# martinambrus/PitchExtractor

Measured on AMD Instinct MI355X. Metric: mel-frames/sec training throughput (JDCNet, 24 kHz, batch=256), higher is better.
Workload: dtype f32

## Files before the change

### pitchextractor_amd/csrc/conv.hip

```cpp
#include <type_traits>
#include "splitk.h"

namespace {
using namespace pe;
typedef unsigned int u32x4_t __attribute__((ext_vector_type(4)));
typedef unsigned int u32x2_t __attribute__((ext_vector_type(2)));

__global__ void repack3x3_kernel(const float* __restrict__ w, float* __restrict__ w_fwd,
                                 float* __restrict__ w_dgrad, int Cout, int Cin) {
  const int idx = blockIdx.x * blockDim.x + threadIdx.x;
  if (idx >= Cout * Cin * 9) return;
  const int tap = idx % 9, ci = (idx / 9) % Cin, co = idx / (9 * Cin);
  const float v = w[idx];
  if (w_fwd) w_fwd[((long)co * 9 + tap) * Cin + ci] = v;
  if (w_dgrad) w_dgrad[((long)ci * 9 + (8 - tap)) * Cout + co] = v;
}

__global__ void transpose2d_kernel(const float* __restrict__ in, float* __restrict__ out, int rows, int cols) {
  __shared__ float tile[32][33];
  const int c0 = blockIdx.x * 32, r0 = blockIdx.y * 32;
  for (int i = threadIdx.y; i < 32; i += 8) {
    const int r = r0 + i, c = c0 + threadIdx.x;
    tile[i][threadIdx.x] = (r < rows && c < cols) ? in[(long)r * cols + c] : 0.f;
  }
// ... 62 lines not shown
template <int NT, class TH = __bf16>
__global__ void wfrag_pack_kernel(const float* __restrict__ w, long ld, int N, int K, uint4* __restrict__ out,
                                  const unsigned* __restrict__ amax = nullptr) {
  const long idx = (long)blockIdx.x * blockDim.x + threadIdx.x;
  const int NB32 = (N + 31) >> 5, KB = K >> 4;
  const int lane = (int)(idx & 63);
  const long blk = idx >> 6;
  if (blk >= (long)NB32 * KB) return;
  const int nb = (int)(blk % NB32), kb = (int)(blk / NB32);
  const int n = nb * 32 + (lane & 31), k = kb * 16 + (lane >> 5) * 8;
  float4 v0 = make_float4(0.f, 0.f, 0.f, 0.f), v1 = v0;
  if (n < N) {
    v0 = *reinterpret_cast<const float4*>(w + (long)n * ld + k);
    v1 = *reinterpret_cast<const float4*>(w + (long)n * ld + k + 4);
  }
  uint4* dst = out + ((long)(kb * NB32 + nb) * NT) * 64 + lane;
  if constexpr (NT == 3) {
    const Split3 a = split3(v0), b = split3(v1);
    dst[0] = make_uint4(a.hi.x, a.hi.y, b.hi.x, b.hi.y);
    dst[64] = make_uint4(a.mid.x, a.mid.y, b.mid.x, b.mid.y);
    dst[128] = make_uint4(a.lo.x, a.lo.y, b.lo.x, b.lo.y);
  } else if constexpr (NT == 2) {
    const float sc = h2_scale(*amax);
    const Split2 a = split2(v0, sc), b = split2(v1, sc);
    dst[0] = make_uint4(a.hi.x, a.hi.y, b.hi.x, b.hi.y);
    dst[64] = make_uint4(a.lo.x, a.lo.y, b.lo.x, b.lo.y);
  } else {
    const half4<TH> a = to_half4<TH>(v0), b = to_half4<TH>(v1);
    const uint2 ua = __builtin_bit_cast(uint2, a), ub = __builtin_bit_cast(uint2, b);
    dst[0] = make_uint4(ua.x, ua.y, ub.x, ub.y);
  }
}

template <int BN, int MODE, int PASSES, int D, bool FA2, class TA = float, class TH = __bf16>
__global__ __launch_bounds__(256, 2) void conv3x3_halo_wf_kernel(const TA* __restrict__ x,
                                                                 const uint4* __restrict__ wf, ConvEpiT<TA> ep, int T,
                                                                 int F, int C, int N, int P, int tiles_m,
                                                                 int tiles_n, const unsigned* amax_x,
                                                                 const unsigned* amax_w) {
  constexpr int NT = mode_terms<MODE>();
  using H = term_t<NT, TH>;
  H2Scales hs{1.f, 1.f, 1.f};
  if constexpr (MODE == kSplit2) hs.load(amax_x, amax_w);
  constexpr int TM = 2, TN = BN / 64, WN = BN / 2;
  constexpr int ZR = PASSES * 32;
  constexpr int AIMG = (ZR + 4) * 32;
  constexpr int S = 18 * TN;
  static_assert(S % D == 0 && D >= 2, "the fragment ring wraps at chunk boundaries");
  __shared__ __attribute__((aligned(16))) H As[NT * AIMG];
  const int tid = threadIdx.x, lane = tid & 63, wv = tid >> 6;
  const int wm = wv >> 1, wn = wv & 1, r = lane & 31, h = lane >> 5;
  const int tile = xcd_remap(blockIdx.x, tiles_m * tiles_n);
  const int p0 = (tile / tiles_n) * 128, n0 = (tile % tiles_n) * BN;
  const int WR = 128 + 2 * F + 2;
  const int srow = tid >> 3, piece = tid & 7;
  const int nchunks = C / 32;

  unsigned vbits[TM];
#pragma unroll
  for (int i = 0; i < TM; ++i) {
    const int p = p0 + wm * 64 + i * 32 + r;
    unsigned b = 0;
    if (p < P) {
      const int f = p % F, t = (p / F) % T;
#pragma unroll
      for (int tap = 0; tap < 9; ++tap) {
        const int tt = t + tap / 3 - 1, ff = f + tap % 3 - 1;
        if (tt >= 0 && tt < T && ff >= 0 && ff < F) b |= 1u << tap;
      }
    }
    vbits[i] = b;
  }

  typedef typename RawQuad<TA>::type Raw;
  Raw ra[PASSES];
  const __amdgpu_buffer_rsrc_t xrs = __builtin_amdgcn_make_buffer_rsrc(
      const_cast<TA*>(x), 0, (unsigned)((long)P * C * (long)sizeof(TA)), 0x00020000);
  unsigned voa[PASSES];
#pragma unroll
  for (int ps = 0; ps < PASSES; ++ps) {
    const int wr = ps * 32 + srow;
    const long q = (long)p0 - F - 1 + wr;
    voa[ps] = (wr < WR && q >= 0 && q < P) ? (unsigned)((q * C + piece * 4) * (long)sizeof(TA)) : 0x80000000u;
  }
  auto fetch_a = [&](int cc) {
    const unsigned so = (unsigned)(cc * 32 * (int)sizeof(TA));
#pragma unroll
// ... 138 lines not shown
#pragma unroll
        for (int g = 0; g < 16; ++g) {
          const int row = row0 + i * 32 + (g & 3) + 8 * (g >> 2), col = n0 + wn * WN + j * 32 + r;
          if (row < ep.rows && col < ep.N) {
            TA* d = ep.Y + (long)row * ep.N + col;
            float v = MODE == kSplit2 ? hs.unscale(acc[i][j][g]) : acc[i][j][g];
            if (ep.accumulate) v += ld1(d);
            st1(d, v);
            if (stats) add_stat(j, row, v);
          }
        }
  };
  if (!ep.buffer) epilogue_pointer();
  else if (ep.accumulate) epilogue_buffer(std::true_type{});
  else epilogue_buffer(std::false_type{});
  if (ep.stats) {
#pragma unroll
    for (int j = 0; j < TN; ++j) {
      s1[j] += __shfl_xor(s1[j], 32, 64);
      s2[j] += __shfl_xor(s2[j], 32, 64);
    }
    __syncthreads();
    double* red = reinterpret_cast<double*>(As);
    if (h == 0) {
#pragma unroll
      for (int j = 0; j < TN; ++j) {
        red[(wm * BN + wn * WN + j * 32 + r) * 2] = s1[j];
        red[(wm * BN + wn * WN + j * 32 + r) * 2 + 1] = s2[j];
      }
    }
    __syncthreads();
    const long tile_m = tile / tiles_n;
    for (int c = tid; c < BN; c += 256) {
      if (n0 + c < ep.N) {
        ep.stats[(tile_m * 2) * ep.N + n0 + c] = red[c * 2] + red[(BN + c) * 2];
        ep.stats[(tile_m * 2 + 1) * ep.N + n0 + c] = red[c * 2 + 1] + red[(BN + c) * 2 + 1];
      }
    }
  }
}

template <int BN, class FM, int PASSES, int D, bool FA2, class TA = typename FM::TA>
int launch_conv_halo_wf(const TA* x, const void* wf, TA* y, int B, int T, int F, int C, int N, int accumulate,
                        double* stats, hipStream_t st, const unsigned* amax_x, const unsigned* amax_w) {
  const int P = B * T * F;
  ConvEpiT<TA> ep{y, P, N, accumulate, stats, pe_epilogue_buffer((long)(P + 128) * N * (long)sizeof(TA))};
  const int tm = pe_cdiv(P, 128), tn = pe_cdiv(N, BN);
  hipLaunchKernelGGL((conv3x3_halo_wf_kernel<BN, FM::MODE, PASSES, D, FA2, TA, typename FM::TH>), dim3(tm * tn),
                     dim3(256), 0, st, x, reinterpret_cast<const uint4*>(wf), ep, T, F, C, N, P, tm, tn, amax_x, amax_w);
  PE_LAUNCH_CHECK();
  return PE_OK;
}

static inline size_t pe_wfrag_bytes_host(int N, int K, int terms) { return (size_t)((N + 31) / 32) * (K / 16) * terms * 1024; }

int conv_halo_passes(int F, int N) {
  const int wr = 128 + 2 * F + 2;
  if (wr <= 7 * 32 && N >= 96) return 7;
  if (wr <= 10 * 32 && N <= 64) return 10;
  return 0;
}

template <int BM, int BN>
__global__ __launch_bounds__(256) void conv3x3_wgrad_kernel(const float* __restrict__ dy, const float* __restrict__ x,
                                                            float* __restrict__ ws, int T, int F, int Cin,
                                                            int Cout, int P, int k_per_split, int tiles_n,
                                                            int n_tiles, int n_chunks) {
  __shared__ __attribute__((aligned(16))) float As[kBK * BM];
  __shared__ __attribute__((aligned(16))) float Bs[kBK * BN];
  const int xcd = blockIdx.x & 7, q = blockIdx.x >> 3;
  const int tap = q % 9;
  const int chunk = (q / 9) * 8 + xcd;
  if (chunk >= n_chunks) return;
  const int tile = chunk % n_tiles, split = chunk / n_tiles;
  const int m0 = (tile / tiles_n) * BM, n0 = (tile % tiles_n) * BN;
  const int kb = split * k_per_split;
  const int ke = min(P, kb + k_per_split);
  KRowLoader<BM> al{dy, (long)Cout, Cout, 0};
  ShiftedPixelLoader<BN> bl;
  bl.p = x; bl.T = T; bl.F = F; bl.C = Cin; bl.dt = tap / 3 - 1; bl.df = tap % 3 - 1;
  al.init(m0, kb);
  bl.init(n0, kb);
  f32x16 acc[BM / 64][BN / 64];
  tn_zero_acc<BM, BN>(acc);
  tn_mainloop<BM, BN>(al, bl, kb, ke, As, Bs, acc);
  float* dst = ws + ((long)split * 9 + tap) * Cout * Cin;
  tn_for_each_acc<BM, BN>(acc, [&](int r, int c, float v) {
    const int co = m0 + r, ci = n0 + c;
    if (co < Cout && ci < Cin) dst[(long)co * Cin + ci] = v;
  });
}

template <int DUMMY>
// ... 525 lines not shown
  if ((K & 15) || (ld & 3)) return PE_E_UNSUPPORTED;
  const long threads = (long)((N + 31) / 32) * (K / 16) * 64;
  hipLaunchKernelGGL((wfrag_pack_kernel<TERMS, typename FM::TH>), dim3(pe_cdiv(threads, 256)), dim3(256), 0,
                     pe_stream(stream), w, ld, N, K, reinterpret_cast<uint4*>(out), TERMS == 2 ? amax : nullptr);
  PE_LAUNCH_CHECK();
  return PE_OK;
}

extern "C" int pe_wfrag_pack(int products, const float* w, long ld, int N, int K, const unsigned* amax, void* wfrag,
                             void* stream) {
  return with_form<kTermForms, false>(products, 0, [&](auto f) {
    return wfrag_pack_impl<decltype(f)>(w, ld, N, K, amax, wfrag, stream);
  });
}

extern "C" int pe_conv3x3_wf_supported(int F, int C, int N) {
  return (C % 32) == 0 && conv_halo_passes(F, N) != 0 ? 1 : 0;
}

extern "C" int pe_conv3x3_wf_stat_parts(int B, int T, int F) { return pe_cdiv((long)B * T * F, 128); }

template <class FM, class TA = typename FM::TA>
static int conv3x3_fwd_wf_impl(const TA* x, const void* wfrag, TA* y, int B, int T, int F, int C, int N,
                               int accumulate, double* stats, void* stream, const unsigned* amax_x,
                               const unsigned* amax_w) {
  constexpr int MODE = FM::MODE;
  if (!x || !wfrag || !y || B <= 0 || T <= 0 || F <= 0 || C <= 0 || N <= 0) return PE_E_ARG;
  if ((C % 32) != 0 || (long)B * T * F * (C > N ? C : N) >= (1L << 31)) return PE_E_UNSUPPORTED;
  if ((long)B * T * F * C * (long)sizeof(TA) >= (1L << 31) || (long)pe_wfrag_bytes_host(N, 9 * C, mode_terms<MODE>()) >= (1L << 31))
    return PE_E_UNSUPPORTED;
  if (MODE == kSplit2 && (!amax_x || !amax_w)) return PE_E_ARG;
  hipStream_t st = pe_stream(stream);
  const int passes = conv_halo_passes(F, N);
  if (passes == 10)
    return launch_conv_halo_wf<64, FM, 10, 6, true>(x, wfrag, y, B, T, F, C, N, accumulate, stats, st, amax_x, amax_w);
  if (passes == 7) {
    if (N % 192 == 0 && N % 128 != 0)
      return launch_conv_halo_wf<192, FM, 7, 3, false>(x, wfrag, y, B, T, F, C, N, accumulate, stats, st, amax_x,
                                                       amax_w);
    return launch_conv_halo_wf<128, FM, 7, 3, true>(x, wfrag, y, B, T, F, C, N, accumulate, stats, st, amax_x, amax_w);
  }
  return PE_E_UNSUPPORTED;
}

extern "C" int pe_conv3x3_fwd_wf(int products, int act16, const void* x, const void* wfrag, void* y, int B, int T, int F,
                                 int C, int N, int accumulate, double* bn_partials, const unsigned* amax_x,
                                 const unsigned* amax_w, void* stream) {
  return with_form<kTermForms, true>(products, act16, [&](auto f) {
    using TA = typename decltype(f)::TA;
    return conv3x3_fwd_wf_impl<decltype(f)>(static_cast<const TA*>(x), wfrag, static_cast<TA*>(y), B, T, F, C, N,
                                            accumulate, bn_partials, stream, amax_x, amax_w);
  });
}

extern "C" size_t pe_conv3x3_wgrad_workspace_bytes(int B, int T, int F, int Cin, int Cout) {
  if (Cin == 1) return (size_t)kC1WgradBlocks * 576 * sizeof(float);
  return (size_t)wgrad_plan(B * T * F, Cout, Cin).k.splits * 9 * Cout * Cin * sizeof(float);
}

template <class FM, class TA = typename FM::TA>
static int conv3x3_wgrad_impl(const TA* x, const TA* dy, float* dw_oihw, int B, int T, int F, int Cin,
                              int Cout, float* workspace, size_t workspace_bytes, void* stream,
                              const unsigned* amax_x, const unsigned* amax_dy) {
  constexpr int MODE = FM::MODE;
  using TH = typename FM::TH;
  if (!x || !dy || !dw_oihw || B <= 0 || T <= 0 || F <= 0 || Cin <= 0 || Cout <= 0) return PE_E_ARG;
  if (MODE == kSplit2 && (!amax_x || !amax_dy)) return PE_E_ARG;
  if ((Cin & 3) || (Cout & 3)) return PE_E_UNSUPPORTED;
// ... 114 lines not shown
```

### pitchextractor_amd/csrc/elementwise.hip

```cpp
#include <type_traits>
#include "forms.h"

namespace {
using namespace pe;

constexpr int kMaxPartials = 4096;

template <class F>
__device__ __forceinline__ void column_reduce2(F&& f, long n_pix, int C, double* partial ) {
  extern __shared__ __attribute__((aligned(16))) char smem_raw[];
  double* red = reinterpret_cast<double*>(smem_raw);
  const int quads = C >> 2;
  const int G = 256 / quads;
  const int q = threadIdx.x % quads, g = threadIdx.x / quads;
  double s1[4] = {0, 0, 0, 0}, s2[4] = {0, 0, 0, 0};
  if (g < G) {
    for (long p = (long)blockIdx.x * G + g; p < n_pix; p += (long)gridDim.x * G) {
      float4 a, b;
      f(p, q * 4, a, b);
      s1[0] += a.x; s1[1] += a.y; s1[2] += a.z; s1[3] += a.w;
      s2[0] += b.x; s2[1] += b.y; s2[2] += b.z; s2[3] += b.w;
    }
#pragma unroll
    for (int i = 0; i < 4; ++i) {
      red[(g * 2 + 0) * C + q * 4 + i] = s1[i];
      red[(g * 2 + 1) * C + q * 4 + i] = s2[i];
    }
  }
  __syncthreads();
  for (int i = threadIdx.x; i < 2 * C; i += 256) {
    double s = 0;
    for (int gg = 0; gg < G; ++gg) s += red[gg * 2 * C + i];
    partial[(long)blockIdx.x * 2 * C + i] = s;
  }
}

__device__ __forceinline__ float lrelu(float v, float slope) { return v > 0.f ? v : v * slope; }

template <class TA>
__global__ __launch_bounds__(256) void bn_stats_partial_kernel(const TA* __restrict__ x, long n_pix, int C,
                                                               double* __restrict__ partial) {
  column_reduce2(
      [&](long p, int c, float4& a, float4& b) {
        a = ld4(x + p * C + c);
        b = make_float4(a.x * a.x, a.y * a.y, a.z * a.z, a.w * a.w);
      },
      n_pix, C, partial);
}

__global__ __launch_bounds__(256) void bn_partials_fold_kernel(const double* __restrict__ partial, int nparts, int C2,
                                                               double* __restrict__ out) {
  for (int col = threadIdx.x; col < C2; col += 256) {
    double s = 0.0;
    for (int p = blockIdx.x; p < nparts; p += gridDim.x) s += partial[(long)p * C2 + col];
    out[(long)blockIdx.x * C2 + col] = s;
  }
}

__global__ void bn_stats_finalize_kernel(const double* __restrict__ partial, int nparts, long n_pix, int C,
                                         const float* __restrict__ gamma, const float* __restrict__ beta, float eps,
                                         float momentum, float* __restrict__ running_mean,
                                         float* __restrict__ running_var, float* __restrict__ mean_out,
                                         float* __restrict__ invstd_out, float* __restrict__ scale,
                                         float* __restrict__ shift) {
  const int c = blockIdx.x * 4 + (threadIdx.x >> 6);
  if (c >= C) return;
  const double s1 = pe_wave_strided_sum(partial + c, 2L * C, nparts);
// ... 248 lines not shown
__global__ __launch_bounds__(256) void bn_bwd_apply_kernel(const BnBwdArgs a, const float* __restrict__ c1,
                                                           const float* __restrict__ c2, float* __restrict__ dx,
                                                           unsigned* __restrict__ amax) {
  const int quads = a.C >> 2;
  const long total = a.n_in_pix * quads;
  float am = 0.f;
  for (long i = (long)blockIdx.x * 256 + threadIdx.x; i < total; i += (long)gridDim.x * 256) {
    const int c = (int)(i % quads) * 4;
    const long p = i / quads;
    const float4 dz = dz_quad(a, p, c);
    const float4 v = *reinterpret_cast<const float4*>(a.x + p * a.C + c);
    const float4 mu = *reinterpret_cast<const float4*>(a.mean + c);
    const float4 is = *reinterpret_cast<const float4*>(a.invstd + c);
    const float4 sc = *reinterpret_cast<const float4*>(a.scale + c);
    const float4 k1 = bn_term(c1, c), k2 = bn_term(c2, c);
    float4 o;
    o.x = sc.x * (dz.x - k1.x - (v.x - mu.x) * is.x * k2.x);
    o.y = sc.y * (dz.y - k1.y - (v.y - mu.y) * is.y * k2.y);
    o.z = sc.z * (dz.z - k1.z - (v.z - mu.z) * is.z * k2.z);
    o.w = sc.w * (dz.w - k1.w - (v.w - mu.w) * is.w * k2.w);
    *reinterpret_cast<float4*>(dx + p * a.C + c) = o;
    am = amax4(am, o);
  }
  amax_commit(am, amax);
}

template <int POOL>
struct BnWindow {
  float4 v[POOL], dz[POOL];
  long p0;
  int n;
};

template <int POOL, class TA>
__device__ __forceinline__ void bn_window(const BnBwdArgsT<TA>& a, long item, int nwin, int c, BnWindow<POOL>& w,
                                          const float4& sc, const float4& sh) {
  const int Fout = a.Fin / POOL;
  const long row = item / nwin;
  const int wi = (int)(item - row * nwin);
  const bool real = wi < Fout;
  w.n = real ? POOL : a.Fin - Fout * POOL;
  w.p0 = row * a.Fin + (long)wi * POOL;
  const TA* xp = a.x + w.p0 * a.C + c;
#pragma unroll
  for (int j = 0; j < POOL; ++j) {
    w.v[j] = j < w.n ? ld4(xp + (long)j * a.C) : make_float4(0.f, 0.f, 0.f, 0.f);
    w.dz[j] = make_float4(0.f, 0.f, 0.f, 0.f);
  }
  if (!real) return;
  const float4 dyv = ld4(a.dy + (row * Fout + wi) * a.lddy + a.coff + c);
  const float scv[4] = {sc.x, sc.y, sc.z, sc.w}, shv[4] = {sh.x, sh.y, sh.z, sh.w};
  const float dys[4] = {dyv.x, dyv.y, dyv.z, dyv.w};
#pragma unroll
  for (int ch = 0; ch < 4; ++ch) {
    float best = lrelu(fmaf(reinterpret_cast<const float*>(&w.v[0])[ch], scv[ch], shv[ch]), a.slope);
    int arg = 0;
#pragma unroll
    for (int j = 1; j < POOL; ++j) {
      const float act = lrelu(fmaf(reinterpret_cast<const float*>(&w.v[j])[ch], scv[ch], shv[ch]), a.slope);
      if (act > best) { best = act; arg = j; }
    }
    const float g = best > 0.f ? dys[ch] : dys[ch] * a.slope;
#pragma unroll
    for (int j = 0; j < POOL; ++j) reinterpret_cast<float*>(&w.dz[j])[ch] = j == arg ? g : 0.f;
  }
}

template <int POOL, class TA>
__global__ __launch_bounds__(256) void bn_bwd_partial_win_kernel(const BnBwdArgsT<TA> a, long n_items, int nwin,
                                                                 double* __restrict__ partial) {
  const int c0 = (threadIdx.x % (a.C >> 2)) * 4;
  const float4 mu = *reinterpret_cast<const float4*>(a.mean + c0), is = *reinterpret_cast<const float4*>(a.invstd + c0);
  const float4 sc = *reinterpret_cast<const float4*>(a.scale + c0), sh = *reinterpret_cast<const float4*>(a.shift + c0);
  column_reduce2(
      [&](long item, int c, float4& s, float4& t) {
        BnWindow<POOL> w;
        bn_window<POOL, TA>(a, item, nwin, c, w, sc, sh);
        s = make_float4(0.f, 0.f, 0.f, 0.f);
        t = make_float4(0.f, 0.f, 0.f, 0.f);
#pragma unroll
        for (int j = 0; j < POOL; ++j) {
          s.x += w.dz[j].x; s.y += w.dz[j].y; s.z += w.dz[j].z; s.w += w.dz[j].w;
          t.x += w.dz[j].x * ((w.v[j].x - mu.x) * is.x); t.y += w.dz[j].y * ((w.v[j].y - mu.y) * is.y);
          t.z += w.dz[j].z * ((w.v[j].z - mu.z) * is.z); t.w += w.dz[j].w * ((w.v[j].w - mu.w) * is.w);
        }
      },
      n_items, a.C, partial);
}

template <class TA>
struct BnTapGrad {
  const TA* dy;
  const unsigned char* arg;
  long lddy;
  int coff;
  unsigned nbw;
};

// ... 41 lines not shown
                                                                   const float* __restrict__ c2, TA* __restrict__ dx,
                                                                   unsigned* __restrict__ amax, const BnTapGrad<TA> t) {
  const int quads = a.C >> 2;
  float am = 0.f;
  const int G = 256 / quads, c = (threadIdx.x % quads) * 4, g = threadIdx.x / quads;
  const float4 mu = *reinterpret_cast<const float4*>(a.mean + c), is = *reinterpret_cast<const float4*>(a.invstd + c);
  const float4 sc = *reinterpret_cast<const float4*>(a.scale + c), sh = *reinterpret_cast<const float4*>(a.shift + c);
  const float4 k1 = bn_term(c1, c), k2 = bn_term(c2, c);
  for (long item = (long)blockIdx.x * G + g; g < G && item < n_items; item += (long)gridDim.x * G) {
    BnWindow<POOL> w;
    bn_window<POOL, TA>(a, item, nwin, c, w, sc, sh);
    const unsigned tw = (unsigned)item / t.nbw;
    const int pos0 = (int)((unsigned)item - tw * t.nbw) * POOL;
    const uchar4 ar = *reinterpret_cast<const uchar4*>(t.arg + (long)tw * a.C + c);
    const float4 tg = ld4(t.dy + (long)tw * t.lddy + t.coff + c);
#pragma unroll
    for (int j = 0; j < POOL; ++j) {
      if (j >= w.n) break;
      float4 o;
      o.x = sc.x * (w.dz[j].x - k1.x - (w.v[j].x - mu.x) * is.x * k2.x);
      o.y = sc.y * (w.dz[j].y - k1.y - (w.v[j].y - mu.y) * is.y * k2.y);
      o.z = sc.z * (w.dz[j].z - k1.z - (w.v[j].z - mu.z) * is.z * k2.z);
      o.w = sc.w * (w.dz[j].w - k1.w - (w.v[j].w - mu.w) * is.w * k2.w);
      am = amax4(am, o);
      const int pj = pos0 + j;
      if (ar.x == pj) { o.x = add_unfused(round_act(dx, o.x), tg.x); am = fmaxf(am, fabsf(o.x)); }
      if (ar.y == pj) { o.y = add_unfused(round_act(dx, o.y), tg.y); am = fmaxf(am, fabsf(o.y)); }
      if (ar.z == pj) { o.z = add_unfused(round_act(dx, o.z), tg.z); am = fmaxf(am, fabsf(o.z)); }
      if (ar.w == pj) { o.w = add_unfused(round_act(dx, o.w), tg.w); am = fmaxf(am, fabsf(o.w)); }
      st4(dx + (w.p0 + j) * a.C + c, o);
    }
  }
  amax_commit(am, amax);
}

template <class TA>
__global__ __launch_bounds__(256) void maxpool_fwd_kernel(const TA* __restrict__ x, TA* __restrict__ y,
                                                          long n_out_pix, int Fin, int C, int pool, long ldy,
                                                          int coff, unsigned char* __restrict__ arg) {
  const int quads = C >> 2, Fout = Fin / pool;
  const long total = n_out_pix * quads;
  for (long i = (long)blockIdx.x * 256 + threadIdx.x; i < total; i += (long)gridDim.x * 256) {
    const int q = (int)(i % quads);
    const long op = i / quads, row = op / Fout;
    const int fo = (int)(op % Fout);
    const TA* xp = x + ((row * Fin + (long)fo * pool) * C + q * 4);
    float4 m = ld4(xp);
    int a0 = 0, a1 = 0, a2 = 0, a3 = 0;
    int j = 1;
    for (; j + 4 <= pool; j += 4) {
      float4 v[4];
#pragma unroll
      for (int u = 0; u < 4; ++u) v[u] = ld4(xp + (long)(j + u) * C);
#pragma unroll
      for (int u = 0; u < 4; ++u) {
        if (v[u].x > m.x) { m.x = v[u].x; a0 = j + u; }
        if (v[u].y > m.y) { m.y = v[u].y; a1 = j + u; }
        if (v[u].z > m.z) { m.z = v[u].z; a2 = j + u; }
        if (v[u].w > m.w) { m.w = v[u].w; a3 = j + u; }
      }
    }
    for (; j < pool; ++j) {
      const float4 v = ld4(xp + (long)j * C);
      if (v.x > m.x) { m.x = v.x; a0 = j; }
      if (v.y > m.y) { m.y = v.y; a1 = j; }
      if (v.z > m.z) { m.z = v.z; a2 = j; }
// ... 125 lines not shown
__global__ __launch_bounds__(256) void copy2d_kernel(const TA* __restrict__ src, long lds, TA* __restrict__ dst,
                                                     long ldd, long rows, int cols, int accumulate) {
  const int quads = cols >> 2;
  const long total = rows * quads;
  for (long i = (long)blockIdx.x * 256 + threadIdx.x; i < total; i += (long)gridDim.x * 256) {
    const int c = (int)(i % quads) * 4;
    const long r = i / quads;
    float4 v = ld4(src + r * lds + c);
    TA* d = dst + r * ldd + c;
    if (accumulate) { const float4 o = ld4(d); v.x += o.x; v.y += o.y; v.z += o.z; v.w += o.w; }
    st4(d, v);
  }
}

int ew_grid(long total_threads) {
  long g = (total_threads + 255) / 256;
  if (g > 16384) g = 16384;
  if (g < 1) g = 1;
  return (int)g;
}

int reduce_grid(long n_pix, int C, int cap = 1024) {
  const int G = 256 / (C / 4);
  long g = (n_pix + G - 1) / G;
  if (g > cap) g = cap;
  if (g < 1) g = 1;
  return (int)g;
}

size_t reduce_lds(int C) { return (size_t)(256 / (C / 4)) * 2 * C * sizeof(double); }

bool bn_channels_ok(int C) { return C >= 4 && (C % 4) == 0 && C <= 1024; }

__global__ __launch_bounds__(256) void absmax_kernel(const float* __restrict__ x, long rows, int cols4, long ld,
                                                     unsigned* __restrict__ out) {
  const long n4 = rows * cols4;
  unsigned m = 0u;
  for (long i = (long)blockIdx.x * 256 + threadIdx.x; i < n4; i += (long)gridDim.x * 256) {
    const long r = i / cols4;
    const int c = (int)(i - r * cols4);
    const float4 v = *reinterpret_cast<const float4*>(x + r * ld + c * 4);
    m = max(m, __float_as_uint(v.x) & 0x7fffffffu);
    m = max(m, __float_as_uint(v.y) & 0x7fffffffu);
    m = max(m, __float_as_uint(v.z) & 0x7fffffffu);
    m = max(m, __float_as_uint(v.w) & 0x7fffffffu);
  }
#pragma unroll
  for (int off = 32; off > 0; off >>= 1) m = max(m, (unsigned)__shfl_xor((int)m, off, 64));
  __shared__ unsigned red[4];
  if ((threadIdx.x & 63) == 0) red[threadIdx.x >> 6] = m;
  __syncthreads();
  if (threadIdx.x == 0) atomicMax(out, max(max(red[0], red[1]), max(red[2], red[3])));
}

__global__ __launch_bounds__(256) void absmax_segments_kernel(const float* __restrict__ base,
                                                              const long* __restrict__ seg_off,
                                                              const long* __restrict__ seg_len,
                                                              unsigned* __restrict__ out) {
  const float* x = base + seg_off[blockIdx.y];
  const long n = seg_len[blockIdx.y];
  unsigned m = 0u;
  for (long i = (long)blockIdx.x * 256 + threadIdx.x; i < n; i += (long)gridDim.x * 256)
    m = max(m, __float_as_uint(x[i]) & 0x7fffffffu);
#pragma unroll
  for (int off = 32; off > 0; off >>= 1) m = max(m, (unsigned)__shfl_xor((int)m, off, 64));
  __shared__ unsigned red[4];
// ... 49 lines not shown
  int n = nparts;
  if (nparts > 512) {
    constexpr int kFold = 512;
    if (!workspace || workspace_bytes < (size_t)kFold * 2 * C * sizeof(double)) return PE_E_WORKSPACE;
    double* folded = reinterpret_cast<double*>(workspace);
    hipLaunchKernelGGL(bn_partials_fold_kernel, dim3(kFold), dim3(256), 0, st, partials, nparts, 2 * C, folded);
    PE_LAUNCH_CHECK();
    src = folded;
    n = kFold;
  }
  hipLaunchKernelGGL(bn_stats_finalize_kernel, dim3(pe_cdiv(C, 4)), dim3(256), 0, st, src, n, n_pix, C, gamma, beta,
                     eps, momentum, running_mean, running_var, mean, invstd, scale, shift);
  PE_LAUNCH_CHECK();
  return PE_OK;
}

extern "C" int pe_bn_eval_affine(const float* gamma, const float* beta, const float* running_mean,
                                 const float* running_var, float eps, int C, float* scale, float* shift,
                                 float* mean, float* invstd, void* stream) {
  if (!gamma || !beta || !running_mean || !running_var || !scale || !shift || !mean || !invstd || C <= 0)
    return PE_E_ARG;
  hipLaunchKernelGGL(bn_eval_affine_kernel, dim3(pe_cdiv(C, 64)), dim3(64), 0, pe_stream(stream), gamma, beta,
                     running_mean, running_var, eps, C, scale, shift, mean, invstd);
  PE_LAUNCH_CHECK();
  return PE_OK;
}

template <class TA>
static int bn_act_pool_fwd_impl(const TA* x, const float* scale, const float* shift, float slope, TA* y, long rows,
                                int Fin, int C, int pool, long ldy, int coff, unsigned* amax_out, void* stream) {
  if (!x || !scale || !shift || !y || rows <= 0 || Fin <= 0 || pool <= 0) return PE_E_ARG;
  if (!bn_channels_ok(C) || (ldy & 3) || (coff & 3)) return PE_E_UNSUPPORTED;
  const long n_out = rows * (Fin / pool);
  hipLaunchKernelGGL(bn_act_pool_fwd_kernel<TA>, dim3(ew_grid(pe_cdiv(n_out, 256 / (C / 4)) * 256L)), dim3(256), 0, pe_stream(stream), x,
                     scale, shift, slope, y, n_out, Fin, C, pool, ldy, coff, amax_out);
  PE_LAUNCH_CHECK();
  return PE_OK;
}

extern "C" int pe_bn_act_pool_fwd(int act16, const void* x, const float* scale, const float* shift, float slope, void* y,
                                  long rows, int Fin, int C, int pool, long ldy, int coff, unsigned* amax_out,
                                  void* stream) {
  return with_act(act16, [&](auto a) {
    using TA = typename decltype(a)::TA;
    return bn_act_pool_fwd_impl(static_cast<const TA*>(x), scale, shift, slope, static_cast<TA*>(y), rows, Fin, C, pool,
                                ldy, coff, amax_out, stream);
  });
}

template <class TA>
static int bn_act_pool_bwd_impl(const TA* x, const TA* dy, const float* scale, const float* shift, const float* mean,
                                const float* invstd, float slope, TA* dx, float* dgamma, float* dbeta, long rows,
                                int Fin, int C, int pool, long lddy, int coff, int eval_mode, void* workspace,
                                size_t workspace_bytes, unsigned* amax_out, void* stream,
                                const BnTapGrad<TA>* tap = nullptr) {
  const bool sums = !(eval_mode && !dgamma && !dbeta);
  if (!x || !dy || !scale || !shift || !mean || !invstd || !dx || rows <= 0) return PE_E_ARG;
  if (sums && (!dgamma || !dbeta)) return PE_E_ARG;
  if (!bn_channels_ok(C) || (lddy & 3) || (coff & 3) || pool <= 0) return PE_E_UNSUPPORTED;
  const size_t need = pe_bn_workspace_bytes(C) + 2 * (size_t)C * sizeof(float);
  if (sums && (!workspace || workspace_bytes < need)) return PE_E_WORKSPACE;
  hipStream_t st = pe_stream(stream);
  BnBwdArgsT<TA> a{x, dy, scale, shift, mean, invstd, slope, rows * Fin, Fin, C, pool, lddy, coff};
  double* partial = reinterpret_cast<double*>(workspace);
  float* c1 = eval_mode ? nullptr
                        : reinterpret_cast<float*>(reinterpret_cast<char*>(workspace) + pe_bn_workspace_bytes(C));
  float* c2 = eval_mode ? nullptr : c1 + C;
  const int nwin = Fin / pool + (Fin % pool ? 1 : 0);
  const long n_items = rows * nwin;
  const bool win = pool == 1 || pool == 2 || pool == 4;
  if (!win && !std::is_same<TA, float>::value) return PE_E_UNSUPPORTED;
  const int grid = reduce_grid(win ? n_items : a.n_in_pix, C,
                               (!std::is_same<TA, float>::value && pool == 1) ? kMaxPartials : 1024);
  if (sums) {
    if (pool == 1)
      hipLaunchKernelGGL((bn_bwd_partial_win_kernel<1, TA>), dim3(grid), dim3(256), reduce_lds(C), st, a, n_items, nwin, partial);
    else if (pool == 2)
      hipLaunchKernelGGL((bn_bwd_partial_win_kernel<2, TA>), dim3(grid), dim3(256), reduce_lds(C), st, a, n_items, nwin, partial);
    else if (pool == 4)
      hipLaunchKernelGGL((bn_bwd_partial_win_kernel<4, TA>), dim3(grid), dim3(256), reduce_lds(C), st, a, n_items, nwin, partial);
    else if constexpr (std::is_same<TA, float>::value)
      hipLaunchKernelGGL(bn_bwd_partial_kernel, dim3(grid), dim3(256), reduce_lds(C), st, a, partial);
    PE_LAUNCH_CHECK();
    hipLaunchKernelGGL(bn_bwd_finalize_kernel, dim3(pe_cdiv(C, 4)), dim3(256), 0, st, partial, grid, a.n_in_pix, C,
                       dgamma, dbeta, c1, c2);
    PE_LAUNCH_CHECK();
  }
  const int agrid = win ? ew_grid(pe_cdiv(n_items, 256 / (C / 4)) * 256L) : ew_grid(a.n_in_pix * (C / 4));
  if (tap != nullptr) {
    if (pool == 1)
      hipLaunchKernelGGL((bn_bwd_apply_win_tap_kernel<1, TA>), dim3(agrid), dim3(256), 0, st, a, n_items, nwin, c1, c2,
                         dx, amax_out, *tap);
    else if (pool == 2)
      hipLaunchKernelGGL((bn_bwd_apply_win_tap_kernel<2, TA>), dim3(agrid), dim3(256), 0, st, a, n_items, nwin, c1, c2,
                         dx, amax_out, *tap);
    else
      hipLaunchKernelGGL((bn_bwd_apply_win_tap_kernel<4, TA>), dim3(agrid), dim3(256), 0, st, a, n_items, nwin, c1, c2,
                         dx, amax_out, *tap);
  } else if (pool == 1)
    hipLaunchKernelGGL((bn_bwd_apply_win_kernel<1, TA>), dim3(agrid), dim3(256), 0, st, a, n_items, nwin, c1, c2, dx,
                       amax_out);
  else if (pool == 2)
    hipLaunchKernelGGL((bn_bwd_apply_win_kernel<2, TA>), dim3(agrid), dim3(256), 0, st, a, n_items, nwin, c1, c2, dx,
                       amax_out);
  else if (pool == 4)
    hipLaunchKernelGGL((bn_bwd_apply_win_kernel<4, TA>), dim3(agrid), dim3(256), 0, st, a, n_items, nwin, c1, c2, dx,
                       amax_out);
  else if constexpr (std::is_same<TA, float>::value)
    hipLaunchKernelGGL(bn_bwd_apply_kernel, dim3(agrid), dim3(256), 0, st, a, c1, c2, dx, amax_out);
// ... 229 lines not shown
```

Measured before the change: 641,100.

## Add 256-pixel halo conv tile and load-ahead BN forward/backward kernels

Adds a PM=256 pixel-tile variant of the halo conv3x3 forward kernel with a wider zone (14 passes), selected by a heuristic for large problems with two or fewer terms. Each block then does more work and reloads the halo less often, at the cost of more LDS and different occupancy. It also adds unrolled load-ahead kernels for BN+activation forward (pool=1) and BN backward partial sums (pool=2), which issue several loads before computing to hide memory latency. Env vars can force the old paths.

```diff
diff --git a/pitchextractor_amd/csrc/conv.hip b/pitchextractor_amd/csrc/conv.hip
--- a/pitchextractor_amd/csrc/conv.hip
+++ b/pitchextractor_amd/csrc/conv.hip
@@ -118,7 +118,7 @@
   }
 }
 
-template <int BN, int MODE, int PASSES, int D, bool FA2, class TA = float, class TH = __bf16>
+template <int BN, int MODE, int PASSES, int D, bool FA2, class TA = float, class TH = __bf16, int PM = 128>
 __global__ __launch_bounds__(256, 2) void conv3x3_halo_wf_kernel(const TA* __restrict__ x,
                                                                  const uint4* __restrict__ wf, ConvEpiT<TA> ep, int T,
                                                                  int F, int C, int N, int P, int tiles_m,
@@ -128,17 +128,19 @@
   using H = term_t<NT, TH>;
   H2Scales hs{1.f, 1.f, 1.f};
   if constexpr (MODE == kSplit2) hs.load(amax_x, amax_w);
-  constexpr int TM = 2, TN = BN / 64, WN = BN / 2;
+  constexpr int WMS = PM / 64, WNS = 4 / WMS;
+  constexpr int TM = 2, WN = BN / WNS, TN = WN / 32;
+  static_assert((PM == 128 || PM == 256) && PM + 2 <= PASSES * 32, "pixel tile");
   constexpr int ZR = PASSES * 32;
   constexpr int AIMG = (ZR + 4) * 32;
   constexpr int S = 18 * TN;
   static_assert(S % D == 0 && D >= 2, "the fragment ring wraps at chunk boundaries");
   __shared__ __attribute__((aligned(16))) H As[NT * AIMG];
   const int tid = threadIdx.x, lane = tid & 63, wv = tid >> 6;
-  const int wm = wv >> 1, wn = wv & 1, r = lane & 31, h = lane >> 5;
+  const int wm = wv / WNS, wn = wv % WNS, r = lane & 31, h = lane >> 5;
   const int tile = xcd_remap(blockIdx.x, tiles_m * tiles_n);
-  const int p0 = (tile / tiles_n) * 128, n0 = (tile % tiles_n) * BN;
-  const int WR = 128 + 2 * F + 2;
+  const int p0 = (tile / tiles_n) * PM, n0 = (tile % tiles_n) * BN;
+  const int WR = PM + 2 * F + 2;
   const int srow = tid >> 3, piece = tid & 7;
   const int nchunks = C / 32;
 
@@ -343,21 +345,26 @@
     __syncthreads();
     const long tile_m = tile / tiles_n;
     for (int c = tid; c < BN; c += 256) {
-      if (n0 + c < ep.N) {
-        ep.stats[(tile_m * 2) * ep.N + n0 + c] = red[c * 2] + red[(BN + c) * 2];
-        ep.stats[(tile_m * 2 + 1) * ep.N + n0 + c] = red[c * 2 + 1] + red[(BN + c) * 2 + 1];
-      }
-    }
-  }
-}
-
-template <int BN, class FM, int PASSES, int D, bool FA2, class TA = typename FM::TA>
+#pragma unroll
+      for (int hf = 0; hf < WMS / 2; ++hf) {
+        const long part = tile_m * (WMS / 2) + hf;
+        if (n0 + c < ep.N && (WMS == 2 || part * 128 < P)) {
+          const double* rh = red + (2 * hf * BN + c) * 2;
+          ep.stats[(part * 2) * ep.N + n0 + c] = rh[0] + rh[BN * 2];
+          ep.stats[(part * 2 + 1) * ep.N + n0 + c] = rh[1] + rh[BN * 2 + 1];
+        }
+      }
+    }
+  }
+}
+
+template <int BN, class FM, int PASSES, int D, bool FA2, int PM = 128, class TA = typename FM::TA>
 int launch_conv_halo_wf(const TA* x, const void* wf, TA* y, int B, int T, int F, int C, int N, int accumulate,
                         double* stats, hipStream_t st, const unsigned* amax_x, const unsigned* amax_w) {
   const int P = B * T * F;
-  ConvEpiT<TA> ep{y, P, N, accumulate, stats, pe_epilogue_buffer((long)(P + 128) * N * (long)sizeof(TA))};
-  const int tm = pe_cdiv(P, 128), tn = pe_cdiv(N, BN);
-  hipLaunchKernelGGL((conv3x3_halo_wf_kernel<BN, FM::MODE, PASSES, D, FA2, TA, typename FM::TH>), dim3(tm * tn),
+  ConvEpiT<TA> ep{y, P, N, accumulate, stats, pe_epilogue_buffer((long)(P + PM) * N * (long)sizeof(TA))};
+  const int tm = pe_cdiv(P, PM), tn = pe_cdiv(N, BN);
+  hipLaunchKernelGGL((conv3x3_halo_wf_kernel<BN, FM::MODE, PASSES, D, FA2, TA, typename FM::TH, PM>), dim3(tm * tn),
                      dim3(256), 0, st, x, reinterpret_cast<const uint4*>(wf), ep, T, F, C, N, P, tm, tn, amax_x, amax_w);
   PE_LAUNCH_CHECK();
   return PE_OK;
@@ -370,6 +377,16 @@
   if (wr <= 7 * 32 && N >= 96) return 7;
   if (wr <= 10 * 32 && N <= 64) return 10;
   return 0;
+}
+
+bool conv_halo_tile256(int terms, long P, int N) {
+  static const int forced = [] {
+    const char* e = getenv("PE_CONV_TILE");
+    return e ? atoi(e) : 0;
+  }();
+  if (terms > 2) return false;
+  if (forced == 128 || forced == 256) return forced == 256;
+  return (long)pe_cdiv(P, 128) * pe_cdiv(N, 64) >= 4 * 512;
 }
 
 template <int BM, int BN>
@@ -961,8 +978,14 @@
   if (MODE == kSplit2 && (!amax_x || !amax_w)) return PE_E_ARG;
   hipStream_t st = pe_stream(stream);
   const int passes = conv_halo_passes(F, N);
-  if (passes == 10)
+  if (passes == 10) {
+    if constexpr (mode_terms<MODE>() <= 2) {
+      if (conv_halo_tile256(mode_terms<MODE>(), (long)B * T * F, N))
+        return launch_conv_halo_wf<64, FM, 14, mode_terms<MODE>() == 2 ? 4 : 6, mode_terms<MODE>() != 2, 256>(
+            x, wfrag, y, B, T, F, C, N, accumulate, stats, st, amax_x, amax_w);
+    }
     return launch_conv_halo_wf<64, FM, 10, 6, true>(x, wfrag, y, B, T, F, C, N, accumulate, stats, st, amax_x, amax_w);
+  }
   if (passes == 7) {
     if (N % 192 == 0 && N % 128 != 0)
       return launch_conv_halo_wf<192, FM, 7, 3, false>(x, wfrag, y, B, T, F, C, N, accumulate, stats, st, amax_x,
diff --git a/pitchextractor_amd/csrc/elementwise.hip b/pitchextractor_amd/csrc/elementwise.hip
--- a/pitchextractor_amd/csrc/elementwise.hip
+++ b/pitchextractor_amd/csrc/elementwise.hip
@@ -6,10 +6,30 @@
 
 constexpr int kMaxPartials = 4096;
 
+__device__ __forceinline__ void column_reduce2_fold(const double (&s1)[4], const double (&s2)[4], int C,
+                                                    double* partial ) {
+  extern __shared__ __attribute__((aligned(16))) char smem_raw[];
+  double* red = reinterpret_cast<double*>(smem_raw);
+  const int quads = C >> 2;
+  const int G = 256 / quads;
+  const int q = threadIdx.x % quads, g = threadIdx.x / quads;
+  if (g < G) {
+#pragma unroll
+    for (int i = 0; i < 4; ++i) {
+      red[(g * 2 + 0) * C + q * 4 + i] = s1[i];
+      red[(g * 2 + 1) * C + q * 4 + i] = s2[i];
+    }
+  }
+  __syncthreads();
+  for (int i = threadIdx.x; i < 2 * C; i += 256) {
+    double s = 0;
+    for (int gg = 0; gg < G; ++gg) s += red[gg * 2 * C + i];
+    partial[(long)blockIdx.x * 2 * C + i] = s;
+  }
+}
+
 template <class F>
 __device__ __forceinline__ void column_reduce2(F&& f, long n_pix, int C, double* partial ) {
-  extern __shared__ __attribute__((aligned(16))) char smem_raw[];
-  double* red = reinterpret_cast<double*>(smem_raw);
   const int quads = C >> 2;
   const int G = 256 / quads;
   const int q = threadIdx.x % quads, g = threadIdx.x / quads;
@@ -21,18 +41,8 @@
       s1[0] += a.x; s1[1] += a.y; s1[2] += a.z; s1[3] += a.w;
       s2[0] += b.x; s2[1] += b.y; s2[2] += b.z; s2[3] += b.w;
     }
-#pragma unroll
-    for (int i = 0; i < 4; ++i) {
-      red[(g * 2 + 0) * C + q * 4 + i] = s1[i];
-      red[(g * 2 + 1) * C + q * 4 + i] = s2[i];
-    }
-  }
-  __syncthreads();
-  for (int i = threadIdx.x; i < 2 * C; i += 256) {
-    double s = 0;
-    for (int gg = 0; gg < G; ++gg) s += red[gg * 2 * C + i];
-    partial[(long)blockIdx.x * 2 * C + i] = s;
-  }
+  }
+  column_reduce2_fold(s1, s2, C, partial);
 }
 
 __device__ __forceinline__ float lrelu(float v, float slope) { return v > 0.f ? v : v * slope; }
@@ -347,6 +357,26 @@
   int n;
 };
 
+template <int POOL>
+__device__ __forceinline__ void bn_window_dz(const float4 (&v)[POOL], const float4& dyv, const float4& sc,
+                                             const float4& sh, float slope, float4 (&dz)[POOL]) {
+  const float scv[4] = {sc.x, sc.y, sc.z, sc.w}, shv[4] = {sh.x, sh.y, sh.z, sh.w};
+  const float dys[4] = {dyv.x, dyv.y, dyv.z, dyv.w};
+#pragma unroll
+  for (int ch = 0; ch < 4; ++ch) {
+    float best = lrelu(fmaf(reinterpret_cast<const float*>(&v[0])[ch], scv[ch], shv[ch]), slope);
+    int arg = 0;
+#pragma unroll
+    for (int j = 1; j < POOL; ++j) {
+      const float act = lrelu(fmaf(reinterpret_cast<const float*>(&v[j])[ch], scv[ch], shv[ch]), slope);
+      if (act > best) { best = act; arg = j; }
+    }
+    const float g = best > 0.f ? dys[ch] : dys[ch] * slope;
+#pragma unroll
+    for (int j = 0; j < POOL; ++j) reinterpret_cast<float*>(&dz[j])[ch] = j == arg ? g : 0.f;
+  }
+}
+
 template <int POOL, class TA>
 __device__ __forceinline__ void bn_window(const BnBwdArgsT<TA>& a, long item, int nwin, int c, BnWindow<POOL>& w,
                                           const float4& sc, const float4& sh) {
@@ -364,21 +394,7 @@
   }
   if (!real) return;
   const float4 dyv = ld4(a.dy + (row * Fout + wi) * a.lddy + a.coff + c);
-  const float scv[4] = {sc.x, sc.y, sc.z, sc.w}, shv[4] = {sh.x, sh.y, sh.z, sh.w};
-  const float dys[4] = {dyv.x, dyv.y, dyv.z, dyv.w};
-#pragma unroll
-  for (int ch = 0; ch < 4; ++ch) {
-    float best = lrelu(fmaf(reinterpret_cast<const float*>(&w.v[0])[ch], scv[ch], shv[ch]), a.slope);
-    int arg = 0;
-#pragma unroll
-    for (int j = 1; j < POOL; ++j) {
-      const float act = lrelu(fmaf(reinterpret_cast<const float*>(&w.v[j])[ch], scv[ch], shv[ch]), a.slope);
-      if (act > best) { best = act; arg = j; }
-    }
-    const float g = best > 0.f ? dys[ch] : dys[ch] * a.slope;
-#pragma unroll
-    for (int j = 0; j < POOL; ++j) reinterpret_cast<float*>(&w.dz[j])[ch] = j == arg ? g : 0.f;
-  }
+  bn_window_dz<POOL>(w.v, dyv, sc, sh, a.slope, w.dz);
 }
 
 template <int POOL, class TA>
@@ -486,6 +502,112 @@
     }
   }
   amax_commit(am, amax);
+}
+
+template <int U, class TA>
+__global__ __launch_bounds__(256) void bn_act_fwd_ahead_kernel(const TA* __restrict__ x, const float* __restrict__ scale,
+                                                               const float* __restrict__ shift, float slope,
+                                                               TA* __restrict__ y, long n_pix, int C, long ldy, int coff,
+                                                               unsigned* __restrict__ amax) {
+  const int quads = C >> 2;
+  float am = 0.f;
+  const int G = 256 / quads, q = threadIdx.x % quads, g = threadIdx.x / quads;
+  const float4 sc = *reinterpret_cast<const float4*>(scale + q * 4), sh = *reinterpret_cast<const float4*>(shift + q * 4);
+  const long step = (long)gridDim.x * G;
+  for (long op = (long)blockIdx.x * G + g; g < G && op < n_pix; op += U * step) {
+    float4 v[U];
+#pragma unroll
+    for (int u = 0; u < U; ++u)
+      if (op + u * step < n_pix) v[u] = ld4(x + ((op + u * step) * C + q * 4));
+#pragma unroll
+    for (int u = 0; u < U; ++u) {
+      const long o = op + u * step;
+      if (o < n_pix) {
+        float4 m;
+        m.x = lrelu(fmaf(v[u].x, sc.x, sh.x), slope);
+        m.y = lrelu(fmaf(v[u].y, sc.y, sh.y), slope);
+        m.z = lrelu(fmaf(v[u].z, sc.z, sh.z), slope);
+        m.w = lrelu(fmaf(v[u].w, sc.w, sh.w), slope);
+        st4(y + o * ldy + coff + q * 4, m);
+        am = amax4(am, m);
+      }
+    }
+  }
+  amax_commit(am, amax);
+}
+
+struct ItemCursor {
+  long row, step_row;
+  int w, step_w, nwin;
+  __device__ __forceinline__ ItemCursor(long item, long step, int nwin_) : nwin(nwin_) {
+    row = item / nwin;
+    w = (int)(item - row * nwin);
+    step_row = step / nwin;
+    step_w = (int)(step - step_row * nwin);
+  }
+  __device__ __forceinline__ void advance() {
+    row += step_row;
+    w += step_w;
+    if (w >= nwin) { w -= nwin; ++row; }
+  }
+};
+
+template <int POOL>
+struct BnWindowIn {
+  float4 v[POOL], dyv;
+  bool real;
+
+  template <class TA>
+  __device__ __forceinline__ void load(const BnBwdArgsT<TA>& a, const ItemCursor& cur, int c) {
+    const int Fout = a.Fin / POOL;
+    real = cur.w < Fout;
+    const int n = real ? POOL : a.Fin - Fout * POOL;
+    const TA* xp = a.x + (cur.row * a.Fin + (long)cur.w * POOL) * a.C + c;
+#pragma unroll
+    for (int j = 0; j < POOL; ++j) v[j] = j < n ? ld4(xp + (long)j * a.C) : make_float4(0.f, 0.f, 0.f, 0.f);
+    if (real) dyv = ld4(a.dy + (cur.row * Fout + cur.w) * a.lddy + a.coff + c);
+  }
+};
+
+template <int POOL, int U, class TA>
+__global__ __launch_bounds__(256) void bn_bwd_partial_ahead_kernel(const BnBwdArgsT<TA> a, long n_items, int nwin,
+                                                                   double* __restrict__ partial) {
+  const int quads = a.C >> 2;
+  const int G = 256 / quads, c = (threadIdx.x % quads) * 4, g = threadIdx.x / quads;
+  const float4 mu = *reinterpret_cast<const float4*>(a.mean + c), is = *reinterpret_cast<const float4*>(a.invstd + c);
+  const float4 sc = *reinterpret_cast<const float4*>(a.scale + c), sh = *reinterpret_cast<const float4*>(a.shift + c);
+  double s1[4] = {0, 0, 0, 0}, s2[4] = {0, 0, 0, 0};
+  const long first = (long)blockIdx.x * G + g, step = (long)gridDim.x * G;
+  if (g < G && first < n_items) {
+    ItemCursor cur(first, step, nwin);
+    for (long item = first; item < n_items; item += U * step) {
+      BnWindowIn<POOL> in[U];
+#pragma unroll
+      for (int u = 0; u < U; ++u) {
+        if (item + u * step < n_items) in[u].load(a, cur, c);
+        cur.advance();
+      }
+#pragma unroll
+      for (int u = 0; u < U; ++u) {
+        if (item + u * step < n_items) {
+          float4 dz[POOL];
+#pragma unroll
+          for (int j = 0; j < POOL; ++j) dz[j] = make_float4(0.f, 0.f, 0.f, 0.f);
+          if (in[u].real) bn_window_dz<POOL>(in[u].v, in[u].dyv, sc, sh, a.slope, dz);
+          float4 s = make_float4(0.f, 0.f, 0.f, 0.f), t = make_float4(0.f, 0.f, 0.f, 0.f);
+#pragma unroll
+          for (int j = 0; j < POOL; ++j) {
+            s.x += dz[j].x; s.y += dz[j].y; s.z += dz[j].z; s.w += dz[j].w;
+            t.x += dz[j].x * ((in[u].v[j].x - mu.x) * is.x); t.y += dz[j].y * ((in[u].v[j].y - mu.y) * is.y);
+            t.z += dz[j].z * ((in[u].v[j].z - mu.z) * is.z); t.w += dz[j].w * ((in[u].v[j].w - mu.w) * is.w);
+          }
+          s1[0] += s.x; s1[1] += s.y; s1[2] += s.z; s1[3] += s.w;
+          s2[0] += t.x; s2[1] += t.y; s2[2] += t.z; s2[3] += t.w;
+        }
+      }
+    }
+  }
+  column_reduce2_fold(s1, s2, a.C, partial);
 }
 
 template <class TA>
@@ -677,6 +799,14 @@
 
 bool bn_channels_ok(int C) { return C >= 4 && (C % 4) == 0 && C <= 1024; }
 
+bool bn_passes_ahead() {
+  static const bool parent = [] {
+    const char* e = getenv("PE_BN_PASSES");
+    return e && strcmp(e, "parent") == 0;
+  }();
+  return !parent;
+}
+
 __global__ __launch_bounds__(256) void absmax_kernel(const float* __restrict__ x, long rows, int cols4, long ld,
                                                      unsigned* __restrict__ out) {
   const long n4 = rows * cols4;
@@ -792,8 +922,14 @@
   if (!x || !scale || !shift || !y || rows <= 0 || Fin <= 0 || pool <= 0) return PE_E_ARG;
   if (!bn_channels_ok(C) || (ldy & 3) || (coff & 3)) return PE_E_UNSUPPORTED;
   const long n_out = rows * (Fin / pool);
-  hipLaunchKernelGGL(bn_act_pool_fwd_kernel<TA>, dim3(ew_grid(pe_cdiv(n_out, 256 / (C / 4)) * 256L)), dim3(256), 0, pe_stream(stream), x,
-                     scale, shift, slope, y, n_out, Fin, C, pool, ldy, coff, amax_out);
+  const dim3 grid(ew_grid(pe_cdiv(n_out, 256 / (C / 4)) * 256L));
+  hipStream_t st = pe_stream(stream);
+  if (pool == 1 && bn_passes_ahead())
+    hipLaunchKernelGGL((bn_act_fwd_ahead_kernel<4, TA>), grid, dim3(256), 0, st, x, scale, shift, slope, y, n_out, C, ldy,
+                       coff, amax_out);
+  else
+    hipLaunchKernelGGL(bn_act_pool_fwd_kernel<TA>, grid, dim3(256), 0, st, x, scale, shift, slope, y, n_out, Fin, C,
+                       pool, ldy, coff, amax_out);
   PE_LAUNCH_CHECK();
   return PE_OK;
 }
@@ -835,6 +971,9 @@
   if (sums) {
     if (pool == 1)
       hipLaunchKernelGGL((bn_bwd_partial_win_kernel<1, TA>), dim3(grid), dim3(256), reduce_lds(C), st, a, n_items, nwin, partial);
+    else if (pool == 2 && bn_passes_ahead())
+      hipLaunchKernelGGL((bn_bwd_partial_ahead_kernel<2, 2, TA>), dim3(grid), dim3(256), reduce_lds(C), st, a, n_items,
+                         nwin, partial);
     else if (pool == 2)
       hipLaunchKernelGGL((bn_bwd_partial_win_kernel<2, TA>), dim3(grid), dim3(256), reduce_lds(C), st, a, n_items, nwin, partial);
     else if (pool == 4)
```

Measured after the change: 644,000, median of 6. About the same (+0.5%).
